# linghuaj/AlphaGo

Measured on AMD Instinct MI355X. Metric: SL-policy positions/sec (whole node) + top-1 move acc, 19x19 12-layer net, higher is better.
Workload: dtype bf16; 1 GPU; model=SL policy net (12-layer, 192 filters, 48 planes), global_batch=2176, per_gpu_batch=2176, seq_len=361, parallelism=dp1, backend=hip, graph=False, wgrad_direct=False, merged_reduce=False

## Files before the change

alphago_amd/_build.py:

```python
from __future__ import annotations

import glob
import hashlib
import os
import subprocess
import sys
import sysconfig
from concurrent.futures import ThreadPoolExecutor

PKG = os.path.dirname(os.path.abspath(__file__))
CSRC = os.path.join(PKG, "csrc")
BUILD = os.path.join(os.path.dirname(PKG), "build", "native")
ROCM = os.environ.get("ROCM_PATH", "/opt/rocm")
ARCH = os.environ.get("PYTORCH_ROCM_ARCH", "gfx950")


def _ext_suffix() -> str:
    return sysconfig.get_config_var("EXT_SUFFIX") or ".so"


def engine_path() -> str:
    return os.path.join(PKG, "_engine" + _ext_suffix())


# ... 75 lines not shown
    return out


def build_selftest(sanitize: str = "", force: bool = False, verbose: bool = False) -> str:
    srcs = sorted(glob.glob(os.path.join(CSRC, "engine", "*.cpp")))
    srcs = [s for s in srcs if not s.endswith(("bindings.cpp", "lzf.cpp", "lockstep.cpp"))]
    hdrs = sorted(glob.glob(os.path.join(CSRC, "engine", "*.h")))
    main = os.path.join(CSRC, "tools", "engine_selftest.cpp")
    tag = sanitize.replace(",", "_") if sanitize else "plain"
    out = os.path.join(BUILD, "engine_selftest_" + tag)
    flags = ["-std=c++17", "-g", "-mpopcnt", "-DAG_NO_PYBIND=1", "-Wall", "-Wno-sign-compare"]
    flags += (["-O1", "-fno-omit-frame-pointer", "-fsanitize=" + sanitize] if sanitize else ["-O2"])
    if sanitize and "undefined" in sanitize:
        flags.append("-fno-sanitize-recover=undefined")
    digest = _digest(srcs + hdrs + [main], " ".join(flags))
    if not force and _up_to_date(out, digest):
        return out
    os.makedirs(BUILD, exist_ok=True)
    _run(["g++", *flags, "-I" + os.path.join(CSRC, "engine"), *srcs, main, "-o", out, "-lpthread"], verbose)
    _write_stamp(out, digest)
    return out


def _torch_paths():
    import torch
    from torch.utils import cpp_extension

    incs = cpp_extension.include_paths(device_type="cuda")
    libdir = os.path.join(os.path.dirname(torch.__file__), "lib")
    abi = "1" if torch._C._GLIBCXX_USE_CXX11_ABI else "0"
    return incs, libdir, abi


def build_hip(force: bool = False, verbose: bool = False, flavor: str = "prod") -> str:
    srcs = _hip_sources(flavor)
    hdrs = sorted(glob.glob(os.path.join(CSRC, "kernels", "*.h")) + [os.path.join(CSRC, "engine", "ladder_bb.h")])
    out = hip_path(flavor)
    incs, libdir, abi = _torch_paths()
    common = [
        "-O3",
        "-std=c++17",
        "-fPIC",
        "-D_GLIBCXX_USE_CXX11_ABI=" + abi,
        "-DUSE_ROCM=1",
        "-D__HIP_PLATFORM_AMD__=1",
        "-DTORCH_EXTENSION_NAME=_hip_kernels",
        "-Wno-unused-result",
        "-Wno-deprecated-declarations",
    ] + {"prod": [], "debug": ["-DAGK_DEBUG=1"],
         "lab": ["-DAGK_KERNEL_LAB=1", "-Dagk=agk_lab", "-Dagk_ops=agk_lab_ops"]}[flavor]
    hip_flags = ["--offload-arch=" + ARCH, "-fgpu-rdc" if False else "-fno-gpu-rdc", "-munsafe-fp-atomics"]
    digest = _digest(srcs + hdrs, " ".join(common + hip_flags))
    if not force and _up_to_date(out, digest):
        return out
    os.makedirs(BUILD, exist_ok=True)
    inc_flags = ["-I" + p for p in incs] + ["-I" + os.path.join(CSRC, "kernels"), "-I" + sysconfig.get_paths()["include"]]
    hipcc = os.path.join(ROCM, "bin", "hipcc")

    def compile_one(src):
        obj = os.path.join(BUILD, "hip_%s_%s.o" % (flavor, os.path.basename(src)))
        cmd = [hipcc, "-x", "hip", *common, *hip_flags, *inc_flags, "-c", src, "-o", obj]
        _run(cmd, verbose)
        return obj

    with ThreadPoolExecutor(max_workers=min(8, max(1, len(srcs)))) as ex:
        objs = list(ex.map(compile_one, srcs))
    tmp = out + ".tmp"
    _run(
        [
            hipcc,
            "-shared",
            "--offload-arch=" + ARCH,
            "-o",
            tmp,
            *objs,
            "-L" + libdir,
            "-Wl,-rpath," + libdir,
            "-lc10",
            "-lc10_hip",
            "-ltorch",
            "-ltorch_cpu",
            "-ltorch_hip",
            "-lamdhip64",
        ],
        verbose,
    )
    os.replace(tmp, out)
    _write_stamp(out, digest)
    return out
# ... 24 lines not shown
```

alphago_amd/csrc/kernels/conv_common.h:

```cpp
#pragma once
#include <hip/hip_runtime.h>

#include <utility>

#include "common.h"
#include "kernels.h"

namespace agk {

#ifdef AGK_DEBUG
static __device__ unsigned g_dbg_err;
#define AGK_DCHECK(cond, code) \
  ((cond) ? true : (atomicOr(&::agk::g_dbg_err, (unsigned)(code)), false))
#else
#define AGK_DCHECK(cond, code) true
#endif
enum : unsigned {
  DBG_FWD_X = 1u << 0,
  DBG_FWD_W = 1u << 1,
  DBG_FWD_Y = 1u << 2,
  DBG_WG_X = 1u << 3,
  DBG_WG_DZ = 1u << 4,
};

// ... 94 lines not shown
  static_assert(OFF >= 0 && OFF < 65536, "ds_read offset: 16-bit unsigned");
  bf16x4 v;
  asm volatile("ds_read_b64_tr_b16 %0, %1 offset:%2" : "=v"(v) : "v"(lds_addr), "n"(OFF));
  return v;
}
template <int OFF = 0>
__device__ __forceinline__ bf16x4 ds_read_tr16_asm(const char* p) {
  return ds_read_tr16_at<OFF>((uint32_t)(uintptr_t)(AG_LDS(p)));
}

__device__ __forceinline__ const char* sgpr_ptr(const char* p) {
  const uint64_t v = (uint64_t)(uintptr_t)p;
  uint32_t lo = __builtin_amdgcn_readfirstlane((uint32_t)v), hi = __builtin_amdgcn_readfirstlane((uint32_t)(v >> 32));
  asm("" : "+s"(lo), "+s"(hi));
  return (const char*)(uintptr_t)(((uint64_t)hi << 32) | lo);
}
__device__ __forceinline__ void glds16_so(const void* sbase, uint32_t voff, void* lds_wave_base) {
  glds16((const char*)sbase + (size_t)voff, lds_wave_base);
}


template <int NB, int MB, int MODE>
struct ConvEpilogue {
  static constexpr int BASE = MODE & 3;
  static constexpr bool RES = (MODE & MODE_RES) != 0;
  static_assert(!RES || BASE == MODE_BIAS_RELU || BASE == MODE_MASKBITS, "skip operand: bias + ReLU or bitmask dgrad");
  static constexpr bool BF8 = BASE == MODE_MASKBITS && !RES;
  static constexpr int RG = !(RES && MB >= 6) ? 1 : (18 / NB < 1 ? 1 : (18 / NB > MB ? MB : 18 / NB));
  int ooff[MB];
  int pix[MB];
  f32x4 bb[NB];
  bf16x4 mk[NB][MB];
  uint32_t mw[MB];
  int mslot, mwords;

  __device__ __forceinline__ void load(const ConvFwdArgs& a, int mrow, int nbase, int wn = 0) {
    const int SS = a.S * a.S;
    mslot = blockIdx.y * 8 + wn * 4 + ((threadIdx.x & 63) >> 4);
    mwords = gridDim.y * 8;
#pragma unroll
    for (int j = 0; j < MB; ++j) {
      int m = mrow + j * 16;
      m = m < a.M ? m : a.M - 1;
      const int b = fdiv(m, a.divSS);
      const int rem = m - b * SS;
      const int ii = fdiv(rem, a.divS);
      const int jj = rem - ii * a.S;
      pix[j] = (b * a.HPo + ii + a.Po) * a.HPo + jj + a.Po;
      ooff[j] = pix[j] * a.Cout + nbase;
    }
    if constexpr (BASE == MODE_BIAS_RELU) {
#pragma unroll
      for (int i = 0; i < NB; ++i) bb[i] = *(const f32x4*)(a.bias + nbase + i * 16);
    } else if constexpr (BASE == MODE_MASK) {
#pragma unroll
      for (int j = 0; j < MB; ++j)
#pragma unroll
        for (int i = 0; i < NB; ++i) mk[i][j] = *(const bf16x4*)(a.mask + ooff[j] + i * 16);
    } else if constexpr (BASE == MODE_MASKBITS) {
#pragma unroll
      for (int j = 0; j < MB; ++j) mw[j] = a.mbits_in[(size_t)pix[j] * mwords + mslot];
    }
  }

  __device__ __forceinline__ void store(const ConvFwdArgs& a, const f32x4 (&acc)[NB][MB], int mrow) const {
    float gmax = 0.f;
    const float gsc = (BF8 && a.y_bf8) ? *a.bf8_scale : 0.f;
    bf16x4 rs[RG][RES ? NB : 1];
#pragma unroll
    for (int j = 0; j < MB; ++j) {
      if constexpr (RES) {
        if (j % RG == 0) {
#pragma unroll
          for (int jg = 0; jg < RG; ++jg)
#pragma unroll
            for (int i = 0; i < NB; ++i)
              if (j + jg < MB) rs[jg][i] = *(const bf16x4*)(a.res + ooff[j + jg < MB ? j + jg : j] + i * 16);
        }
      }
      if (mrow + j * 16 >= a.M) continue;
      uint32_t bits = 0u;
#pragma unroll
      for (int i = 0; i < NB; ++i) {
        f32x4 v = acc[i][j];
        if constexpr (RES) {
#pragma unroll
          for (int r = 0; r < 4; ++r)
            v[r] = (BASE == MODE_BIAS_RELU ? v[r] + bb[i][r] : v[r]) + (float)rs[j % RG][i][r];
        }
        if constexpr (BASE == MODE_BIAS_RELU && RES) {
          v[0] = fmaxf(v[0], 0.f);
          v[1] = fmaxf(v[1], 0.f);
          v[2] = fmaxf(v[2], 0.f);
          v[3] = fmaxf(v[3], 0.f);
        } else if constexpr (BASE == MODE_BIAS_RELU) {
          v[0] = fmaxf(v[0] + bb[i][0], 0.f);
          v[1] = fmaxf(v[1] + bb[i][1], 0.f);
          v[2] = fmaxf(v[2] + bb[i][2], 0.f);
          v[3] = fmaxf(v[3] + bb[i][3], 0.f);
        } else if constexpr (BASE == MODE_MASK) {
          v[0] = (float)mk[i][j][0] > 0.f ? v[0] : 0.f;
          v[1] = (float)mk[i][j][1] > 0.f ? v[1] : 0.f;
          v[2] = (float)mk[i][j][2] > 0.f ? v[2] : 0.f;
          v[3] = (float)mk[i][j][3] > 0.f ? v[3] : 0.f;
        } else if constexpr (BASE == MODE_MASKBITS) {
#pragma unroll
          for (int r = 0; r < 4; ++r) v[r] = ((mw[j] >> (4 * i + r)) & 1u) ? v[r] : 0.f;
        }
        bf16x4 o;
        o[0] = (__bf16)v[0];
        o[1] = (__bf16)v[1];
        o[2] = (__bf16)v[2];
        o[3] = (__bf16)v[3];
        if constexpr (BASE == MODE_BIAS_RELU) {
#pragma unroll
          for (int r = 0; r < 4; ++r) bits |= ((float)o[r] > 0.f ? 1u : 0u) << (4 * i + r);
        }
#ifdef AGK_DEBUG
        const long long yo = (long long)ooff[j] + i * 16;
        if (AGK_DCHECK(yo >= 0 && yo + 4 <= a.y_elems, DBG_FWD_Y)) *(bf16x4*)(a.y + yo) = o;
#else
        *(bf16x4*)(a.y + ooff[j] + i * 16) = o;
#endif
        if constexpr (BF8) {
          if (a.y_bf8) {
            float sv[4];
#pragma unroll
            for (int r = 0; r < 4; ++r) {
              gmax = fmaxf(gmax, fabsf(v[r]));
              sv[r] = fminf(fmaxf(v[r] * gsc, -57344.f), 57344.f);
            }
            int pk = __builtin_amdgcn_cvt_pk_bf8_f32(sv[0], sv[1], 0, false);
            pk = __builtin_amdgcn_cvt_pk_bf8_f32(sv[2], sv[3], pk, true);
            *(int*)(a.y_bf8 + ooff[j] + i * 16) = pk;
          }
        }
      }
      if constexpr (BASE == MODE_BIAS_RELU)
        if (a.mbits_out) a.mbits_out[(size_t)pix[j] * mwords + mslot] = bits;
    }
    if constexpr (BF8) {
      if (a.y_bf8 && a.bf8_amax) {
        gmax = wave_max(gmax);
        if ((threadIdx.x & 63) == 0 && gmax > 0.f) atomicMax(a.bf8_amax + (blockIdx.x & 63), __float_as_uint(gmax));
      }
    }
  }
};

template <int NB, int MB, int MODE>
__device__ __forceinline__ void conv_store_tile(const ConvFwdArgs& a, const f32x4 (&acc)[NB][MB], int mrow,
                                                int nbase, int wn) {
  ConvEpilogue<NB, MB, MODE> ep;
  ep.load(a, mrow, nbase, wn);
  ep.store(a, acc, mrow);
}

template <int NB, int MB, int MODE>
struct ConvEpilogue32 {
  static constexpr int BASE = MODE & 3;
  static constexpr bool RES = (MODE & MODE_RES) != 0;
  static_assert(!RES || BASE == MODE_BIAS_RELU || BASE == MODE_MASKBITS, "skip operand: bias + ReLU or bitmask dgrad");
  int ooff[MB];
  int pix[MB];
  f32x4 bb[NB][4];
  bf16x4 mk[NB][MB][4];
  uint2 mw[MB];
  int mslot, mwords;

  __device__ __forceinline__ void load(const ConvFwdArgs& a, int mrow, int nbase, int wn) {
    const int SS = a.S * a.S;
    const int h = (threadIdx.x & 63) >> 5;
    mslot = blockIdx.y * 8 + wn * 4 + h;
    mwords = gridDim.y * 8;
#pragma unroll
    for (int j = 0; j < MB; ++j) {
      int m = mrow + j * 32;
      m = m < a.M ? m : a.M - 1;
      const int b = fdiv(m, a.divSS);
      const int rem = m - b * SS;
      const int ii = fdiv(rem, a.divS);
      const int jj = rem - ii * a.S;
      pix[j] = (b * a.HPo + ii + a.Po) * a.HPo + jj + a.Po;
      ooff[j] = pix[j] * a.Cout + nbase + 4 * h;
    }
    if constexpr (BASE == MODE_BIAS_RELU) {
#pragma unroll
// ... 76 lines not shown
```

alphago_amd/csrc/kernels/conv_fwd_variants.hip:

```cpp
#include <hip/hip_runtime.h>

#include <algorithm>
#include <numeric>

#include "common.h"
#include "conv_common.h"
#include "kernels.h"

namespace agk {

constexpr int HALO_BM = 256;
constexpr int HALO_ROWS = 320;
constexpr int HALO_PW = HALO_ROWS / 8 / 8;


template <int BN, int MODE>
__global__ __launch_bounds__(512, 1) void conv_fwd_halo_kernel(ConvFwdArgs a) {
  constexpr int NB = BN / 32;
  constexpr int MB = 4;
  constexpr int W_BYTES = BN * 128;
  constexpr int H_BYTES = HALO_ROWS * 128;
  constexpr int NW_PW = BN / 64;
  extern __shared__ __attribute__((aligned(16))) char smem[];
  char* const hbuf = smem;
// ... 387 lines not shown
    asm volatile("s_waitcnt lgkmcnt(0)" ::: "memory");
    if constexpr (STAMP) ts[3] = __builtin_amdgcn_s_memtime();
    __builtin_amdgcn_sched_barrier(0);
    __builtin_amdgcn_s_barrier();
    __builtin_amdgcn_sched_barrier(0);
    if constexpr (STAMP) ts[4] = __builtin_amdgcn_s_memtime();
    __builtin_amdgcn_s_setprio(1);
#pragma unroll
    for (int i = 0; i < NB; ++i)
#pragma unroll
      for (int j = 0; j < MB; ++j) acc[i][j] = mfma16x16x32(wf[i], xf[j], acc[i][j]);
    __builtin_amdgcn_s_setprio(0);
    __builtin_amdgcn_sched_barrier(0);
    if constexpr (STAMP) ts[5] = __builtin_amdgcn_s_memtime();
    __builtin_amdgcn_s_barrier();
    __builtin_amdgcn_sched_barrier(0);
    if constexpr (STAMP) {
      ts[6] = __builtin_amdgcn_s_memtime();
#pragma unroll
      for (int i = 0; i < 6; ++i) st_sum[i] += ts[i + 1] - ts[i];
      st_sum[6] += ts[7] - ts[0];
    }
  }
  if constexpr (STAMP) {
    if (lane == 0) {
      unsigned long long* d = a.dbg + ((size_t)blockIdx.x * 8 + wave) * 8;
#pragma unroll
      for (int i = 0; i < 6; ++i) d[i] = st_sum[i];
      d[6] = __builtin_amdgcn_s_memtime() - st_begin;
      d[7] = nK | (st_sum[6] << 16);
    }
  }
  if (grp == 0) __builtin_amdgcn_s_barrier();
  ep.store(a, acc, ep_mrow);
}


template <int BN, int MODE>
static void launch_fwd_pp(const ConvFwdArgs& a_in, hipStream_t st) {
  constexpr int smem = PP_SLOTS * (PP_BM * 64 + BN * 64);
  if constexpr (BN == 192 && MODE == MODE_BIAS_RELU) {
    if (a_in.dbg) {
      static const hipError_t attr_d = hipFuncSetAttribute((const void*)conv_fwd_pp_kernel<BN, MODE, true>,
                            hipFuncAttributeMaxDynamicSharedMemorySize, smem);
  hip_check(attr_d, "hipFuncSetAttribute(max dynamic LDS)");
      ConvFwdArgs a = a_in;
      dim3 grid((a.M + PP_BM - 1) / PP_BM, a.Cout / BN);
      hipLaunchKernelGGL((conv_fwd_pp_kernel<BN, MODE, true>), grid, dim3(512), smem, st, a);
      return;
    }
  }
  const ConvFwdArgs& a = a_in;
  static const hipError_t attr = hipFuncSetAttribute((const void*)conv_fwd_pp_kernel<BN, MODE>, hipFuncAttributeMaxDynamicSharedMemorySize, smem);
  hip_check(attr, "hipFuncSetAttribute(max dynamic LDS)");
  dim3 grid((a.M + PP_BM - 1) / PP_BM, a.Cout / BN);
  hipLaunchKernelGGL((conv_fwd_pp_kernel<BN, MODE>), grid, dim3(512), smem, st, a);
}

template <int BN, int MODE>
static void launch_fwd_ring(const ConvFwdArgs& a, hipStream_t st) {
  constexpr int smem = RING_SLOTS * (RING_BM * 64 + BN * 64);
  static const hipError_t attr = hipFuncSetAttribute((const void*)conv_fwd_ring_kernel<BN, MODE>, hipFuncAttributeMaxDynamicSharedMemorySize,
                        smem);
  hip_check(attr, "hipFuncSetAttribute(max dynamic LDS)");
  dim3 grid((a.M + RING_BM - 1) / RING_BM, a.Cout / BN);
  hipLaunchKernelGGL((conv_fwd_ring_kernel<BN, MODE>), grid, dim3(512), smem, st, a);
// ... 111 lines not shown
  for (int ks = 0; ks < nK; ++ks) {
    const int tn = (t + 1 == T) ? 0 : t + 1;
    const int cn = (t + 1 == T) ? c + 1 : c;
    if (ks + 1 < nK) stage_w(tn, cn, (ks + 1) & 1);
    if (t == 0 && c + 1 < CC) stage_halo(c + 1, (c + 1) & 1);
    if (ks == (nK > 2 ? nK - 2 : 0)) ep.load(a, ep_mrow, ep_nbase, wn);
    const char* hb = hbuf + (c & 1) * H_BYTES;
    const char* wb = wbuf + (ks & 1) * W_BYTES;
    const int kh = t / a.K, kw = t - (t / a.K) * a.K;
    const int toff = (kh - a.K / 2) * HP + (kw - a.K / 2) + G;
#pragma unroll
    for (int kk = 0; kk < 2; ++kk) {
      const int ch = (kk << 2) + (lane >> 4);
      bf16x8 xf[MB], wf[NB];
#pragma unroll
      for (int j = 0; j < MB; ++j) {
        const int row = qrel[j] + toff - G;
        xf[j] = *(const bf16x8*)(hb + row * 128 + ((ch ^ ((row >> 1) & 7)) << 4));
      }
#pragma unroll
      for (int i = 0; i < NB; ++i) wf[i] = *(const bf16x8*)(wb + wrow0 + i * 16 * 128 + ((ch ^ swzw) << 4));
      __builtin_amdgcn_s_setprio(1);
#pragma unroll
      for (int i = 0; i < NB; ++i)
#pragma unroll
        for (int j = 0; j < MB; ++j) acc[i][j] = mfma16x16x32(wf[i], xf[j], acc[i][j]);
      __builtin_amdgcn_s_setprio(0);
    }
    wait_vmcnt0();
    __syncthreads();
    t = tn;
    c = cn;
  }
  ep.store(a, acc, ep_mrow);
}

template <int BN, int MODE, bool STAMP = false>
__global__ __launch_bounds__(512, 1) void conv_fwd_hpp_kernel(ConvFwdArgs a) {
  uint64_t st_sum[8] = {0, 0, 0, 0, 0, 0, 0, 0}, ts[9];
#define HPP_STAMP(i)                          \
  if constexpr (STAMP) {                      \
    __builtin_amdgcn_sched_barrier(0);        \
    ts[i] = __builtin_amdgcn_s_memtime();     \
    __builtin_amdgcn_sched_barrier(0);        \
  }
  constexpr int NB = BN / 32;
  constexpr int MB = 4;
  constexpr int H_BYTES = HC_ROWS * 128;
  constexpr int W_BYTES = BN * 128;
  constexpr int WP = BN / 32;
  constexpr int H_PIECES = HC_DATA / 8;
  constexpr int HP1 = H_PIECES / 4;
  constexpr int HP_STEP = 2;
  constexpr int T = 9;
  static_assert(HP1 == 5 * HP_STEP && H_PIECES % 8 == 0, "halo pieces must be issued within steps 0..4");
  extern __shared__ __attribute__((aligned(16))) char smem[];
  char* const hbuf = smem;
  char* const wbuf = smem + 2 * H_BYTES;

  const int lane = threadIdx.x & 63;
  const int wave = wave_id();
  const int grp = wave >> 2;
  const int wq = wave & 3;
  const int wm = grp * 2 + ((wave >> 1) & 1);
  const int wn = wave & 1;
  const int nwg = gridDim.x;
// ... 134 lines not shown
    __builtin_amdgcn_sched_group_barrier(0x008, NB * MB - 2 * (MB + NB), 0);
    asm volatile("s_waitcnt lgkmcnt(0)" ::: "memory");
    __builtin_amdgcn_sched_barrier(0);
#pragma unroll
    for (int i = 0; i < NB; ++i)
#pragma unroll
      for (int j = 0; j < MB; ++j) acc[i][j] = mfma16x16x32(wf[1][i], xf[1][j], acc[i][j]);
    __builtin_amdgcn_s_setprio(0);
    HPP_STAMP(5);
    __builtin_amdgcn_sched_barrier(0);
    if (grp == 0) wait_vmcnt0();
    HPP_STAMP(6);
    __builtin_amdgcn_sched_barrier(0);
    __builtin_amdgcn_s_barrier();
    __builtin_amdgcn_sched_barrier(0);
    HPP_STAMP(7);
    if constexpr (STAMP) {
#pragma unroll
      for (int i = 0; i < 7; ++i) st_sum[i] += ts[i + 1] - ts[i];
    }
    t = tn; c = cn; kh = khn; kw = kwn;
    wslot = wslot == 2 ? 0 : wslot + 1;
  }
  if constexpr (STAMP) {
    if (lane == 0) {
      unsigned long long* d = a.dbg + ((size_t)blockIdx.x * 8 + wave) * 8;
#pragma unroll
      for (int i = 0; i < 7; ++i) d[i] = st_sum[i];
      d[7] = __builtin_amdgcn_s_memtime() - st_begin;
    }
  }
#undef HPP_STAMP
  if (grp == 0) __builtin_amdgcn_s_barrier();
  ep.store(a, acc, ep_mrow);
}

constexpr int H32_DATA3 = 320;
constexpr int H32_DATA5 = 344;

template <int BN, int MODE, int K, bool STAMP = false>
__global__ __launch_bounds__(512, 1) void conv_fwd_h32_kernel(ConvFwdArgs a) {
  uint64_t st_sum[8] = {0, 0, 0, 0, 0, 0, 0, 0}, ts[9];
#define H32_STAMP(i)                          \
  if constexpr (STAMP) {                      \
    __builtin_amdgcn_sched_barrier(0);        \
    ts[i] = __builtin_amdgcn_s_memtime();     \
    __builtin_amdgcn_sched_barrier(0);        \
  }
  constexpr int NB = BN / 64;
  constexpr int MB = 2;
  constexpr int T = K * K;
  constexpr int HDATA = K == 3 ? H32_DATA3 : H32_DATA5;
  constexpr int HROWS = HDATA + 16;
  constexpr int NHBUF = K == 3 ? 2 : 1;
  constexpr int H_BYTES = HROWS * 128;
  constexpr int W_BYTES = BN * 128;
  constexpr int WP = BN / 64;
  constexpr int H_PIECES = HDATA / 8;
  constexpr int HP1 = H_PIECES / 4;
  constexpr int HP_STEP = 2;
  static_assert(K == 5 || HP1 == 5 * HP_STEP, "K=3 halo pieces are issued in steps 0..4");
  extern __shared__ __attribute__((aligned(16))) char smem[];
  char* const hbuf = smem;
  char* const wbuf = smem + NHBUF * H_BYTES;

  const int lane = threadIdx.x & 63;
// ... 337 lines not shown
```

alphago_amd/csrc/kernels/conv_kernels.h:

```cpp
#pragma once
#include <hip/hip_runtime.h>

#include <stdexcept>

#include "common.h"
#include "conv_common.h"
#include "kernels.h"

namespace agk {

template <int BN, int MODE, int BM, int MBW, bool EPF = true, bool PIPE = true, bool M32 = false, bool ILV = false,
          bool STR = false, bool CO = false, int NS = 2, bool SK = false>
__global__ __launch_bounds__(BM / MBW * 8, 1) void conv_fwd_kernel(ConvFwdArgs a) {
  constexpr int NW = BM / (16 * MBW) * 2;
  constexpr int NB = BN / 32;
  constexpr int MB = MBW;
  constexpr int A_BYTES = BM * 128;
  constexpr int B_BYTES = BN * 128;
  constexpr int STAGE = A_BYTES + B_BYTES;
  constexpr int A_ROWS_PW = BM / NW;
  constexpr int A_INSTR = A_ROWS_PW / 8;
  constexpr bool BDIST = (BN / NW) % 8 != 0;
  constexpr int B_ROWS_PW = BN / NW;
  constexpr int B_INSTR = BDIST ? (BN / 8 + NW - 1) / NW : B_ROWS_PW / 8;
// ... 137 lines not shown
  auto mfmas = [&](const bf16x8 (&xf)[MB], const bf16x8 (&wf)[NB]) {
#pragma unroll
    for (int i = 0; i < NB; ++i)
#pragma unroll
      for (int j = 0; j < MB; ++j) acc[i][j] = mfma16x16x32(wf[i], xf[j], acc[i][j]);
  };

  bf16x8 xa[MB], wa[NB], xb[MB], wb[NB];
  const int ep_mrow = m0 + wm * 16 * MB + (lane & 15);
  const int ep_nbase = n0 + wn * (BN / 2) + ((lane >> 4) << 2);
  ConvEpilogue<NB, MB, MODE> ep;
  const int ep_at = EPF ? (nK > 2 ? nK - 2 : 0) : nK - 1;
  if constexpr (NS > 2) {
    static_assert(PIPE && !M32 && !ILV && !BDIST, "ring: the pipelined 16x16 loop");
    constexpr int PW = A_INSTR + B_INSTR;
    static_assert(PW * (NS - 2) <= 63, "vmcnt range");
#pragma unroll
    for (int s = 0; s < NS - 1; ++s)
      if (s < nK) stage(s);
    for (int ks = 0; ks < nK; ++ks) {
      const int later = (nK - 1 - ks) < (NS - 2) ? (nK - 1 - ks) : (NS - 2);
      ring_wait<PW, NS - 2>(later);
      __syncthreads();
      if (ks + NS - 1 < nK) stage((ks + NS - 1) % NS);
      const char* base = smem + (ks % NS) * STAGE;
      read_frags(base, 0, xa, wa);
      read_frags(base, 1, xb, wb);
      if (ks == ep_at) ep.load(a, ep_mrow, ep_nbase, wn);
      __builtin_amdgcn_s_setprio(1);
      mfmas(xa, wa);
      mfmas(xb, wb);
      __builtin_amdgcn_s_setprio(0);
    }
    ep.store(a, acc, ep_mrow);
    return;
  }
  if constexpr (SK) {
    static_assert(PIPE && !M32 && !ILV && !CO, "split-K: the pipelined 2-buffer loop, tap-outer order");
    const int z = blockIdx.z, nz = gridDim.z;
    const int kb = (int)((long)nK * z / nz), ke = (int)((long)nK * (z + 1) / nz);
    for (int i = 0; i < kb; ++i) st_advance();
    if (kb < ke) {
      stage(0);
      wait_vmcnt0();
      __syncthreads();
      read_frags(smem, 0, xa, wa);
      for (int ks = kb; ks < ke; ++ks) {
        const int cur = (ks - kb) & 1;
        const char* base = smem + cur * STAGE;
        if (ks + 1 < ke) stage(cur ^ 1);
        read_frags(base, 1, xb, wb);
        __builtin_amdgcn_sched_barrier(0);
        __builtin_amdgcn_s_setprio(1);
        mfmas(xa, wa);
        mfmas(xb, wb);
        __builtin_amdgcn_s_setprio(0);
        __builtin_amdgcn_sched_barrier(0);
        wait_vmcnt0();
        __syncthreads();
        if (ks + 1 < ke) read_frags(smem + (cur ^ 1) * STAGE, 0, xa, wa);
      }
    }
    float* ws = a.sk_ws + (size_t)z * a.M * a.Cout;
#pragma unroll
    for (int j = 0; j < MB; ++j) {
      const int m = ep_mrow + j * 16;
// ... 77 lines not shown
      int xo0, xo1;
      size_t wo0, wo1;
      st_offsets(xo0, xo1, wo0, wo1);
      xo0 = more ? xo0 : lxo0;
      xo1 = more ? xo1 : lxo1;
      wo0 = more ? wo0 : lwo0;
      wo1 = more ? wo1 : lwo1;
      lxo0 = xo0;
      lxo1 = xo1;
      lwo0 = wo0;
      lwo1 = wo1;
      asm volatile("s_waitcnt lgkmcnt(0)" ::: "memory");
      __builtin_amdgcn_sched_barrier(0);
      __builtin_amdgcn_s_setprio(1);
#pragma unroll
      for (int d = 0; d < NDMA; ++d) {
        mfma_range(d * MPD, (d + 1) * MPD);
        __builtin_amdgcn_sched_barrier(0);
        st_piece(d, nb, xo0, xo1, wo0, wo1);
        __builtin_amdgcn_sched_barrier(0);
      }
      mfma_range(NDMA * MPD, NMF);
      __builtin_amdgcn_s_setprio(0);
      __builtin_amdgcn_sched_barrier(0);
      st_advance();
      read_frags(base, 1, xa, wa);
      __builtin_amdgcn_s_setprio(1);
      mfmas(xa, wa);
      __builtin_amdgcn_s_setprio(0);
      wait_vmcnt0();
      __syncthreads();
    }
    ep.load(a, ep_mrow, ep_nbase, wn);
    ep.store(a, acc, ep_mrow);
    return;
  }
  if constexpr (!PIPE) {
    for (int ks = 0; ks < nK; ++ks) {
      const int cur = ks & 1;
      const char* base = smem + cur * STAGE;
      if (ks + 1 < nK) stage(cur ^ 1);
#pragma unroll
      for (int kk = 0; kk < 2; ++kk) {
        read_frags(base, kk, xa, wa);
        __builtin_amdgcn_s_setprio(1);
        mfmas(xa, wa);
        __builtin_amdgcn_s_setprio(0);
      }
      wait_vmcnt0();
      __syncthreads();
    }
    ep.load(a, ep_mrow, ep_nbase, wn);
    ep.store(a, acc, ep_mrow);
    return;
  }
  read_frags(smem, 0, xa, wa);
  for (int ks = 0; ks < nK; ++ks) {
    const int cur = ks & 1;
    const char* base = smem + cur * STAGE;
    if (ks + 1 < nK) stage(cur ^ 1);
    if (ks == ep_at) ep.load(a, ep_mrow, ep_nbase, wn);
    read_frags(base, 1, xb, wb);
    __builtin_amdgcn_sched_barrier(0);
    __builtin_amdgcn_s_setprio(1);
    mfmas(xa, wa);
    mfmas(xb, wb);
    __builtin_amdgcn_s_setprio(0);
    __builtin_amdgcn_sched_barrier(0);
    wait_vmcnt0();
    __syncthreads();
    if (ks + 1 < nK) read_frags(base + (cur ^ 1) * STAGE - cur * STAGE, 0, xa, wa);
  }

  ep.store(a, acc, ep_mrow);
}

template <int BN, int MODE, int BM, int MBW, bool EPF = true, bool PIPE = true, bool M32 = false, bool ILV = false,
          bool STR = false, bool CO = false, int NS = 2>
static void launch_fwd_bm(const ConvFwdArgs& a, hipStream_t st) {
  constexpr int smem = NS * (BM * 128 + BN * 128);
  static_assert(smem <= 160 * 1024, "LDS");
  static const hipError_t attr = hipFuncSetAttribute(
      (const void*)conv_fwd_kernel<BN, MODE, BM, MBW, EPF, PIPE, M32, ILV, STR, CO, NS>,
      hipFuncAttributeMaxDynamicSharedMemorySize, smem);
  hip_check(attr, "hipFuncSetAttribute(max dynamic LDS)");
  dim3 grid((a.M + BM - 1) / BM, a.Cout / BN);
  hipLaunchKernelGGL((conv_fwd_kernel<BN, MODE, BM, MBW, EPF, PIPE, M32, ILV, STR, CO, NS>), grid,
                     dim3(BM / MBW * 8), smem, st, a);
}

constexpr int H384_BM = 384;
constexpr int H384_SMAX = 19;
constexpr int H384_DATA = (H384_BM + 2 * (H384_SMAX + 1) + 7) / 8 * 8;
constexpr int H384_ROWS = H384_DATA + 8;
constexpr int H384_PIECES = H384_DATA / 8;

template <int V>
struct IntC {
  static constexpr int value = V;
};

template <int BN, int MODE>
__global__ __launch_bounds__(512, 1) void conv_fwd_halo384_kernel(ConvFwdArgs a) {
  constexpr int BM = H384_BM, MB = 6, NW = 8;
  constexpr int NB = BN / 32;
  constexpr int NMF = NB * MB;
  constexpr int H_BYTES = H384_ROWS * 128;
  constexpr int W_BYTES = BN * 128;
  constexpr int WP = BN / 8 / NW;
  constexpr int HPW = (H384_PIECES + NW - 1) / NW;
  static_assert(BN % 64 == 0 && BM == NW / 2 * 16 * MB, "tile geometry");
  static_assert(2 * H_BYTES + 2 * W_BYTES <= 160 * 1024, "LDS: two halo buffers and two weight slots, S <= 19");
  static_assert(HPW <= 7, "the next chunk's halo is issued in the first seven taps");
  extern __shared__ __attribute__((aligned(16))) char smem[];
  char* const hbuf = smem;
  char* const wbuf = smem + 2 * H_BYTES;

  const int lane = threadIdx.x & 63;
  const int wave = wave_id();
  const int wm = wave >> 1, wn = wave & 1;
  const int m0 = blockIdx.x * BM;
  const int n0 = blockIdx.y * BN;
  const int S = a.S;
  const int SS = S * S;
  const int CC = a.Cin >> 6;
  const int G = S + 1;
  const int Pc = a.offi + 1;

  int hoff[HPW];
#pragma unroll
  for (int i = 0; i < HPW; ++i) {
    const int k = i * NW + wave < H384_PIECES ? i * NW + wave : H384_PIECES - 1;
    const int r = k * 8 + (lane >> 3);
    int m = m0 - G + r;
    m = m < 0 ? 0 : (m >= a.M ? a.M - 1 : m);
    const int b = fdiv(m, a.divSS);
    const int rem = m - b * SS;
    const int ii = fdiv(rem, a.divS);
    const int q = (b * a.HPi + ii + Pc) * a.HPi + (rem - ii * S) + Pc;
    hoff[i] = q * a.Cin + (((lane & 7) ^ ((r >> 1) & 7)) << 3);
  }
  auto halo_piece = [&](int i, int c, int buf) {
    const int k = i * NW + wave < H384_PIECES ? i * NW + wave : H384_PIECES - 1;
    const int xo = hoff[i] + c * 64;
#ifdef AGK_DEBUG
    const bool ok = AGK_DCHECK(xo >= 0 && (long long)xo + 8 <= a.x_elems, DBG_FWD_X);
    glds16(a.x + (ok ? xo : 0), hbuf + buf * H_BYTES + k * 1024);
#else
    glds16(a.x + xo, hbuf + buf * H_BYTES + k * 1024);
#endif
// ... 95 lines not shown
    }
    mfma_range(NDMA * MPD, NMF);
    __builtin_amdgcn_s_setprio(0);
    __builtin_amdgcn_sched_barrier(0);
#pragma unroll
    for (int j = 0; j < MB; ++j) xa[j] = *(const bf16x8*)(hb + (xo[j] ^ 64));
#pragma unroll
    for (int i = 0; i < NB; ++i) wa[i] = *(const bf16x8*)(wbuf + ws * W_BYTES + (wfrag0 ^ 64) + i * 16 * 128);
    __builtin_amdgcn_s_setprio(1);
    mfma_range(0, NMF);
    __builtin_amdgcn_s_setprio(0);
    wait_vmcnt0();
    __syncthreads();
    ws ^= 1;
  };
  auto chunk = [&](auto nc, int c) {
    step(IntC<0>{}, nc, c);
    step(IntC<1>{}, nc, c);
    step(IntC<2>{}, nc, c);
    step(IntC<3>{}, nc, c);
    step(IntC<4>{}, nc, c);
    step(IntC<5>{}, nc, c);
    step(IntC<6>{}, nc, c);
    step(IntC<7>{}, nc, c);
    step(IntC<8>{}, nc, c);
  };
  for (int c = 0; c + 1 < CC; ++c) chunk(IntC<1>{}, c);
  chunk(IntC<0>{}, CC - 1);

  int ep_mrow = m0 + wm * 16 * MB + pix16;
  asm volatile("" : "+v"(ep_mrow));
  const int ep_nbase = n0 + wn * (BN / 2) + ((lane >> 4) << 2);
  ConvEpilogue<NB, MB, MODE> ep;
  ep.load(a, ep_mrow, ep_nbase, wn);
  ep.store(a, acc, ep_mrow);
}

template <int BN, int MODE>
static bool halo384_covers(const ConvFwdArgs& a) {
  return BN == 192 && ((MODE & 3) == MODE_BIAS_RELU || (MODE & 3) == MODE_MASKBITS) && a.K == 3 && a.Cin % 64 == 0 &&
         a.Cin >= 64 && a.S <= H384_SMAX && a.offi >= 0 && 9ll * a.Cout * a.Cin < (1ll << 31);
}

template <int BN, int MODE>
static void launch_fwd_halo384(const ConvFwdArgs& a, hipStream_t st) {
  if constexpr (BN == 192 && ((MODE & 3) == MODE_BIAS_RELU || (MODE & 3) == MODE_MASKBITS)) {
    constexpr int smem = 2 * H384_ROWS * 128 + 2 * BN * 128;
    static const hipError_t attr = hipFuncSetAttribute((const void*)conv_fwd_halo384_kernel<BN, MODE>,
                                                       hipFuncAttributeMaxDynamicSharedMemorySize, smem);
    hip_check(attr, "hipFuncSetAttribute(max dynamic LDS)");
    dim3 grid((a.M + H384_BM - 1) / H384_BM, a.Cout / BN);
    hipLaunchKernelGGL((conv_fwd_halo384_kernel<BN, MODE>), grid, dim3(512), smem, st, a);
  } else {
    throw std::invalid_argument("conv_fwd: tile 388 is the 192-wide forward / bitmask dgrad");
  }
}

template <int MODE, int NB>
__global__ __launch_bounds__(256) void conv_splitk_finish_kernel(ConvFwdArgs a) {
  constexpr int BN = 32 * NB;
  constexpr int BASE = MODE & 3;
  constexpr bool RES = (MODE & MODE_RES) != 0;
  const int WPP = (a.Cout / BN) * 8;
  const long gid = (long)blockIdx.x * 256 + threadIdx.x;
  if (gid >= (long)a.M * WPP) return;
  const int m = (int)(gid / WPP), w = (int)(gid - (long)m * WPP);
  const int base = (w >> 3) * BN + ((w >> 2) & 1) * (BN / 2) + 4 * (w & 3);
  f32x4 v[NB];
#pragma unroll
  for (int i = 0; i < NB; ++i) v[i] = f32x4{0.f, 0.f, 0.f, 0.f};
  for (int z = 0; z < a.sk_nsplit; ++z) {
    const float* src = a.sk_ws + ((size_t)z * a.M + m) * a.Cout + base;
#pragma unroll
    for (int i = 0; i < NB; ++i) v[i] += *(const f32x4*)(src + 16 * i);
  }
  const int SS = a.S * a.S;
  const int b = fdiv(m, a.divSS);
  const int rem = m - b * SS;
  const int ii = fdiv(rem, a.divS);
  const int jj = rem - ii * a.S;
  const size_t pix = (size_t)(b * a.HPo + ii + a.Po) * a.HPo + jj + a.Po;
  uint32_t mw = 0u, bits = 0u;
  if constexpr (BASE == MODE_MASKBITS) mw = a.mbits_in[pix * WPP + w];
#pragma unroll
// ... 148 lines not shown
  const int swz = (lane & 15) >> 1;
  const int xrow0 = (wm * 16 * MB + (lane & 15)) * 128;
  const int wrow0 = A_BYTES + (wn * (BN / 2) + (lane & 15)) * 128;
  bf16x8 xf[MB], wf[NB];
  ConvEpilogue<NB, MB, MODE_BIAS_RELU> ep;
  const int ep_mrow = m0 + wm * 16 * MB + (lane & 15);
  const int ep_nbase = n0 + wn * (BN / 2) + ((lane >> 4) << 2);

  stage(0);
  wait_vmcnt0();
  __syncthreads();
  for (int ks = 0; ks < nK; ++ks) {
    const int cur = ks & 1;
    const char* base = smem + cur * STAGE;
    if (ks + 1 < nK) stage(cur ^ 1);
#pragma unroll
    for (int kk = 0; kk < 2; ++kk) {
      const int choff = (((kk << 2) + (lane >> 4)) ^ swz) << 4;
#pragma unroll
      for (int j = 0; j < MB; ++j) xf[j] = *(const bf16x8*)(base + xrow0 + j * 16 * 128 + choff);
#pragma unroll
      for (int i = 0; i < NB; ++i) wf[i] = *(const bf16x8*)(base + wrow0 + i * 16 * 128 + choff);
      __builtin_amdgcn_s_setprio(1);
#pragma unroll
      for (int i = 0; i < NB; ++i)
#pragma unroll
        for (int j = 0; j < MB; ++j) acc[i][j] = mfma16x16x32(wf[i], xf[j], acc[i][j]);
      __builtin_amdgcn_s_setprio(0);
    }
    wait_vmcnt0();
    __syncthreads();
  }
  ep.load(a, ep_mrow, ep_nbase, wn);
  ep.store(a, acc, ep_mrow);
}


template <int WN, int WC, int NWC, int TAPS, int NWN = 2>
__device__ __forceinline__ void wgrad_store(const ConvWgradArgs& a,
                                            const f32x4 (&acc)[TAPS][WN / (16 * NWN)][WC / (16 * NWC)],
                                            const float (&dbs)[WN / (16 * NWN)], unsigned bmask, int split, int t,
                                            int n0, int c0, int wn, int wc, int lane, int zero_split) {
  constexpr int NBn = WN / (16 * NWN), NBc = WC / (16 * NWC);
  const int nb0 = n0 + wn * (WN / NWN) + ((lane >> 4) << 2);
  const int cbase = c0 + wc * (WC / NWC) + (lane & 15);
  if (a.grad_w) {
    const float sc = a.scale, be = a.beta;
#pragma unroll
    for (int tp = 0; tp < TAPS; ++tp)
#pragma unroll
      for (int i = 0; i < NBn; ++i)
#pragma unroll
        for (int j = 0; j < NBc; ++j) {
          const int c = cbase + j * 16;
#pragma unroll
          for (int r = 0; r < 4; ++r) {
            const int n = nb0 + i * 16 + r;
            if (n < a.cout_real && c < a.cin_real) {
              float* g = a.grad_w + ((size_t)n * a.cin_real + c) * a.T + t + tp;
              *g = (be != 0.f ? be * *g : 0.f) + sc * acc[tp][i][j][r];
            }
          }
        }
    if (bmask && a.grad_b) {
#pragma unroll
      for (int i = 0; i < NBn; ++i) {
// ... 628 lines not shown
```

alphago_amd/csrc/kernels/conv_lab.hip:

```cpp
#include <hip/hip_runtime.h>

#include "conv_kernels.h"

namespace agk {

template <int BN, int MODE>
__global__ __launch_bounds__(512, 1) void conv_fwd_ga_kernel(ConvFwdArgs a) {
  constexpr int MB = 3;
  constexpr int NB = BN / 16;
  constexpr int NH = NB / 2;
  constexpr int BM = 8 * 16 * MB;
  constexpr int W_BYTES = BN * 128;
  constexpr int WPIECES = BN / 8;
  constexpr int WPW = (WPIECES + 7) / 8;
  static_assert(NB % 2 == 0, "two channel halves");
  extern __shared__ __attribute__((aligned(16))) char smem[];

  const int lane = threadIdx.x & 63;
  const int wave = wave_id();
  const int nwg = gridDim.x;
  const int xcd = blockIdx.x & 7, q8 = nwg >> 3, r8 = nwg & 7;
  const int tile = (xcd < r8 ? xcd * (q8 + 1) : r8 * (q8 + 1) + (xcd - r8) * q8) + (blockIdx.x >> 3);
  const int m0 = tile * BM;
  const int n0 = blockIdx.y * BN;
// ... 82 lines not shown
      const int ch = ((kk << 2) + (lane >> 4)) ^ swz;
#pragma unroll
      for (int h = 0; h < 2; ++h) {
        bf16x8 wf[NH];
#pragma unroll
        for (int i = 0; i < NH; ++i) wf[i] = *(const bf16x8*)(wb + wr0 + (h * NH + i) * 16 * 128 + (ch << 4));
        __builtin_amdgcn_s_setprio(1);
#pragma unroll
        for (int i = 0; i < NH; ++i)
#pragma unroll
          for (int j = 0; j < MB; ++j) acc[h * NH + i][j] = mfma16x16x32(wf[i], x[kk][j], acc[h * NH + i][j]);
        __builtin_amdgcn_s_setprio(0);
      }
      __builtin_amdgcn_sched_barrier(0);
      load_x(x[kk], kk);
      __builtin_amdgcn_sched_barrier(0);
    }
    advance();
    store_w((ks + 1) & 1);
    __syncthreads();
  }
  wait_vmcnt0();

  const int mrow = m0 + wave * 16 * MB + (lane & 15);
#pragma unroll
  for (int h = 0; h < 2; ++h) {
    f32x4 ah[NH][MB];
#pragma unroll
    for (int i = 0; i < NH; ++i)
#pragma unroll
      for (int j = 0; j < MB; ++j) ah[i][j] = acc[h * NH + i][j];
    ConvEpilogue<NH, MB, MODE> ep;
    ep.load(a, mrow, n0 + h * (BN / 2) + ((lane >> 4) << 2), h);
    ep.store(a, ah, mrow);
  }
}

template <int BN, int MODE>
static void launch_fwd_ga(const ConvFwdArgs& a, hipStream_t st) {
  constexpr int smem = 2 * BN * 128;
  static const hipError_t attr = hipFuncSetAttribute((const void*)conv_fwd_ga_kernel<BN, MODE>, hipFuncAttributeMaxDynamicSharedMemorySize, smem);
  hip_check(attr, "hipFuncSetAttribute(max dynamic LDS)");
  constexpr int BM = 8 * 16 * 3;
  dim3 grid((a.M + BM - 1) / BM, a.Cout / BN);
  hipLaunchKernelGGL((conv_fwd_ga_kernel<BN, MODE>), grid, dim3(512), smem, st, a);
}


template <int WN, int WC, int WRING_SLOTS>
__global__ __launch_bounds__(512, 1) void conv_wgrad_ring_kernel(ConvWgradArgs a) {
  constexpr int AHEAD = WRING_SLOTS - 1;
  constexpr int NBn = WN / 32;
  constexpr int NBc = WC / 64;
  constexpr int DZ_BYTES = WN * 64;
  constexpr int X_BYTES = WC * 64;
  constexpr int SLOT = DZ_BYTES + X_BYTES;
  constexpr int NINSTR = (WN + WC) / 16;
  constexpr int IPW = (NINSTR + 7) / 8;
  extern __shared__ __attribute__((aligned(16))) char smem[];

  const int lane = threadIdx.x & 63;
  const int wave = wave_id();
  const int wn = wave >> 2, wc = wave & 3;
  const int split = blockIdx.x;
  const int t = blockIdx.y;
  const int ncb = a.Cin / WC;
// ... 245 lines not shown
```

Measured before the change: 137,300 positions/s.

## Widen conv epilogue stores via permlane16 swap and hoist epilogue branching

The forward conv epilogue now pairs adjacent channel blocks and uses permlane16_swap so each lane writes 16-byte (and 8-byte bf8) stores instead of 8-byte (4-byte) ones, halving store instruction count. Runtime branches on y_bf8/mbits_out are hoisted out of the per-element loop into templated store_rows variants, and a settle() step pins epilogue loads in registers before the store phase (with bf8 scale made scalar via readfirstlane). A lab-only timestamp probe variant of the halo384 kernel is added, plus a build-flag refactor. Risks include extra register pressure and changed store address patterns.

```diff
diff --git a/alphago_amd/_build.py b/alphago_amd/_build.py
--- a/alphago_amd/_build.py
+++ b/alphago_amd/_build.py
@@ -131,10 +131,7 @@
     return incs, libdir, abi
 
 
-def build_hip(force: bool = False, verbose: bool = False, flavor: str = "prod") -> str:
-    srcs = _hip_sources(flavor)
-    hdrs = sorted(glob.glob(os.path.join(CSRC, "kernels", "*.h")) + [os.path.join(CSRC, "engine", "ladder_bb.h")])
-    out = hip_path(flavor)
+def hip_compile_flags(flavor: str = "prod"):
     incs, libdir, abi = _torch_paths()
     common = [
         "-O3",
@@ -149,11 +146,19 @@
     ] + {"prod": [], "debug": ["-DAGK_DEBUG=1"],
          "lab": ["-DAGK_KERNEL_LAB=1", "-Dagk=agk_lab", "-Dagk_ops=agk_lab_ops"]}[flavor]
     hip_flags = ["--offload-arch=" + ARCH, "-fgpu-rdc" if False else "-fno-gpu-rdc", "-munsafe-fp-atomics"]
+    inc_flags = ["-I" + p for p in incs] + ["-I" + os.path.join(CSRC, "kernels"), "-I" + sysconfig.get_paths()["include"]]
+    return common, hip_flags, inc_flags, libdir
+
+
+def build_hip(force: bool = False, verbose: bool = False, flavor: str = "prod") -> str:
+    srcs = _hip_sources(flavor)
+    hdrs = sorted(glob.glob(os.path.join(CSRC, "kernels", "*.h")) + [os.path.join(CSRC, "engine", "ladder_bb.h")])
+    out = hip_path(flavor)
+    common, hip_flags, inc_flags, libdir = hip_compile_flags(flavor)
     digest = _digest(srcs + hdrs, " ".join(common + hip_flags))
     if not force and _up_to_date(out, digest):
         return out
     os.makedirs(BUILD, exist_ok=True)
-    inc_flags = ["-I" + p for p in incs] + ["-I" + os.path.join(CSRC, "kernels"), "-I" + sysconfig.get_paths()["include"]]
     hipcc = os.path.join(ROCM, "bin", "hipcc")
 
     def compile_one(src):
diff --git a/alphago_amd/csrc/kernels/conv_common.h b/alphago_amd/csrc/kernels/conv_common.h
--- a/alphago_amd/csrc/kernels/conv_common.h
+++ b/alphago_amd/csrc/kernels/conv_common.h
@@ -150,6 +150,7 @@
   f32x4 bb[NB];
   bf16x4 mk[NB][MB];
   uint32_t mw[MB];
+  float gsc;
   int mslot, mwords;
 
   __device__ __forceinline__ void load(const ConvFwdArgs& a, int mrow, int nbase, int wn = 0) {
@@ -178,13 +179,105 @@
     } else if constexpr (BASE == MODE_MASKBITS) {
 #pragma unroll
       for (int j = 0; j < MB; ++j) mw[j] = a.mbits_in[(size_t)pix[j] * mwords + mslot];
-    }
-  }
+      if constexpr (BF8) gsc = a.y_bf8 ? *a.bf8_scale : 0.f;
+    }
+  }
+
+  __device__ __forceinline__ void settle() {
+    if constexpr (RES) return;
+    if constexpr (BASE == MODE_BIAS_RELU) {
+#pragma unroll
+      for (int i = 0; i < NB; ++i) asm volatile("" : "+v"(bb[i]));
+    } else if constexpr (BASE == MODE_MASK) {
+#pragma unroll
+      for (int i = 0; i < NB; ++i)
+#pragma unroll
+        for (int j = 0; j < MB; ++j) asm volatile("" : "+v"(mk[i][j]));
+    } else if constexpr (BASE == MODE_MASKBITS) {
+#pragma unroll
+      for (int j = 0; j < MB; ++j) asm volatile("" : "+v"(mw[j]));
+      if constexpr (BF8) {
+        asm volatile("" : "+v"(gsc));
+        gsc = __uint_as_float(__builtin_amdgcn_readfirstlane(__float_as_uint(gsc)));
+      }
+    }
+  }
+
+  static constexpr int NBP = RES ? 0 : NB;
+  typedef uint32_t u32x4_a8 __attribute__((ext_vector_type(4), aligned(8)));
+  typedef uint32_t u32x2_a4 __attribute__((ext_vector_type(2), aligned(4)));
 
   __device__ __forceinline__ void store(const ConvFwdArgs& a, const f32x4 (&acc)[NB][MB], int mrow) const {
     float gmax = 0.f;
-    const float gsc = (BF8 && a.y_bf8) ? *a.bf8_scale : 0.f;
+    if constexpr (BF8) {
+      if (a.y_bf8) store_rows<0, true>(a, acc, mrow, gmax);
+      else store_rows<0, false>(a, acc, mrow, gmax);
+      if (a.y_bf8 && a.bf8_amax) {
+        gmax = wave_max(gmax);
+        if ((threadIdx.x & 63) == 0 && gmax > 0.f) atomicMax(a.bf8_amax + (blockIdx.x & 63), __float_as_uint(gmax));
+      }
+    } else if constexpr (BASE == MODE_BIAS_RELU && RES) {
+      store_rows<2, false>(a, acc, mrow, gmax);
+    } else if constexpr (BASE == MODE_BIAS_RELU) {
+      if (a.mbits_out) store_rows<1, false>(a, acc, mrow, gmax);
+      else store_rows<0, false>(a, acc, mrow, gmax);
+    } else {
+      store_rows<0, false>(a, acc, mrow, gmax);
+    }
+  }
+
+  template <int BITS, bool E5M2>
+  __device__ __forceinline__ void store_rows(const ConvFwdArgs& a, const f32x4 (&acc)[NB][MB], int mrow,
+                                             float& gmax) const {
+    const int po = (threadIdx.x & 16) ? 12 : 0;
     bf16x4 rs[RG][RES ? NB : 1];
+    auto block = [&](int i, int j, uint2& ow, uint32_t& pk, uint32_t& bits) {
+      f32x4 v = acc[i][j];
+      if constexpr (RES) {
+#pragma unroll
+        for (int r = 0; r < 4; ++r)
+          v[r] = (BASE == MODE_BIAS_RELU ? v[r] + bb[i][r] : v[r]) + (float)rs[j % RG][i][r];
+      }
+      if constexpr (BASE == MODE_BIAS_RELU && RES) {
+        v[0] = fmaxf(v[0], 0.f);
+        v[1] = fmaxf(v[1], 0.f);
+        v[2] = fmaxf(v[2], 0.f);
+        v[3] = fmaxf(v[3], 0.f);
+      } else if constexpr (BASE == MODE_BIAS_RELU) {
+        v[0] = fmaxf(v[0] + bb[i][0], 0.f);
+        v[1] = fmaxf(v[1] + bb[i][1], 0.f);
+        v[2] = fmaxf(v[2] + bb[i][2], 0.f);
+        v[3] = fmaxf(v[3] + bb[i][3], 0.f);
+      } else if constexpr (BASE == MODE_MASK) {
+        v[0] = (float)mk[i][j][0] > 0.f ? v[0] : 0.f;
+        v[1] = (float)mk[i][j][1] > 0.f ? v[1] : 0.f;
+        v[2] = (float)mk[i][j][2] > 0.f ? v[2] : 0.f;
+        v[3] = (float)mk[i][j][3] > 0.f ? v[3] : 0.f;
+      } else if constexpr (BASE == MODE_MASKBITS) {
+#pragma unroll
+        for (int r = 0; r < 4; ++r) v[r] = ((mw[j] >> (4 * i + r)) & 1u) ? v[r] : 0.f;
+      }
+      bf16x4 o;
+      o[0] = (__bf16)v[0];
+      o[1] = (__bf16)v[1];
+      o[2] = (__bf16)v[2];
+      o[3] = (__bf16)v[3];
+      if constexpr (BASE == MODE_BIAS_RELU) {
+#pragma unroll
+        for (int r = 0; r < 4; ++r) bits |= ((float)o[r] > 0.f ? 1u : 0u) << (4 * i + r);
+      }
+      ow = __builtin_bit_cast(uint2, o);
+      if constexpr (E5M2) {
+        float sv[4];
+#pragma unroll
+        for (int r = 0; r < 4; ++r) {
+          gmax = fmaxf(gmax, fabsf(v[r]));
+          sv[r] = fminf(fmaxf(v[r] * gsc, -57344.f), 57344.f);
+        }
+        int p = __builtin_amdgcn_cvt_pk_bf8_f32(sv[0], sv[1], 0, false);
+        pk = (uint32_t)__builtin_amdgcn_cvt_pk_bf8_f32(sv[2], sv[3], p, true);
+      }
+    };
 #pragma unroll
     for (int j = 0; j < MB; ++j) {
       if constexpr (RES) {
@@ -199,69 +292,47 @@
       if (mrow + j * 16 >= a.M) continue;
       uint32_t bits = 0u;
 #pragma unroll
-      for (int i = 0; i < NB; ++i) {
-        f32x4 v = acc[i][j];
-        if constexpr (RES) {
-#pragma unroll
-          for (int r = 0; r < 4; ++r)
-            v[r] = (BASE == MODE_BIAS_RELU ? v[r] + bb[i][r] : v[r]) + (float)rs[j % RG][i][r];
+      for (int i = 0; i + 1 < NBP; i += 2) {
+        uint2 o0, o1;
+        uint32_t p0 = 0u, p1 = 0u;
+        block(i, j, o0, p0, bits);
+        block(i + 1, j, o1, p1, bits);
+        const auto sx = __builtin_amdgcn_permlane16_swap(o0.x, o1.x, false, false);
+        const auto sy = __builtin_amdgcn_permlane16_swap(o0.y, o1.y, false, false);
+        u32x4_a8 q;
+        q[0] = sx[0];
+        q[1] = sy[0];
+        q[2] = sx[1];
+        q[3] = sy[1];
+#ifdef AGK_DEBUG
+        const long long yo = (long long)ooff[j] + i * 16 + po;
+        if (AGK_DCHECK(yo >= 0 && yo + 8 <= a.y_elems, DBG_FWD_Y)) *(u32x4_a8*)(a.y + yo) = q;
+#else
+        *(u32x4_a8*)(a.y + ooff[j] + i * 16 + po) = q;
+#endif
+        if constexpr (E5M2) {
+          const auto sp = __builtin_amdgcn_permlane16_swap(p0, p1, false, false);
+          u32x2_a4 q8;
+          q8[0] = sp[0];
+          q8[1] = sp[1];
+          *(u32x2_a4*)(a.y_bf8 + ooff[j] + i * 16 + po) = q8;
         }
-        if constexpr (BASE == MODE_BIAS_RELU && RES) {
-          v[0] = fmaxf(v[0], 0.f);
-          v[1] = fmaxf(v[1], 0.f);
-          v[2] = fmaxf(v[2], 0.f);
-          v[3] = fmaxf(v[3], 0.f);
-        } else if constexpr (BASE == MODE_BIAS_RELU) {
-          v[0] = fmaxf(v[0] + bb[i][0], 0.f);
-          v[1] = fmaxf(v[1] + bb[i][1], 0.f);
-          v[2] = fmaxf(v[2] + bb[i][2], 0.f);
-          v[3] = fmaxf(v[3] + bb[i][3], 0.f);
-        } else if constexpr (BASE == MODE_MASK) {
-          v[0] = (float)mk[i][j][0] > 0.f ? v[0] : 0.f;
-          v[1] = (float)mk[i][j][1] > 0.f ? v[1] : 0.f;
-          v[2] = (float)mk[i][j][2] > 0.f ? v[2] : 0.f;
-          v[3] = (float)mk[i][j][3] > 0.f ? v[3] : 0.f;
-        } else if constexpr (BASE == MODE_MASKBITS) {
-#pragma unroll
-          for (int r = 0; r < 4; ++r) v[r] = ((mw[j] >> (4 * i + r)) & 1u) ? v[r] : 0.f;
-        }
-        bf16x4 o;
-        o[0] = (__bf16)v[0];
-        o[1] = (__bf16)v[1];
-        o[2] = (__bf16)v[2];
-        o[3] = (__bf16)v[3];
-        if constexpr (BASE == MODE_BIAS_RELU) {
-#pragma unroll
-          for (int r = 0; r < 4; ++r) bits |= ((float)o[r] > 0.f ? 1u : 0u) << (4 * i + r);
-        }
+      }
+#pragma unroll
+      for (int i = NBP / 2 * 2; i < NB; ++i) {
+        uint2 o0;
+        uint32_t p0 = 0u;
+        block(i, j, o0, p0, bits);
 #ifdef AGK_DEBUG
         const long long yo = (long long)ooff[j] + i * 16;
-        if (AGK_DCHECK(yo >= 0 && yo + 4 <= a.y_elems, DBG_FWD_Y)) *(bf16x4*)(a.y + yo) = o;
+        if (AGK_DCHECK(yo >= 0 && yo + 4 <= a.y_elems, DBG_FWD_Y)) *(uint2*)(a.y + yo) = o0;
 #else
-        *(bf16x4*)(a.y + ooff[j] + i * 16) = o;
+        *(uint2*)(a.y + ooff[j] + i * 16) = o0;
 #endif
-        if constexpr (BF8) {
-          if (a.y_bf8) {
-            float sv[4];
-#pragma unroll
-            for (int r = 0; r < 4; ++r) {
-              gmax = fmaxf(gmax, fabsf(v[r]));
-              sv[r] = fminf(fmaxf(v[r] * gsc, -57344.f), 57344.f);
-            }
-            int pk = __builtin_amdgcn_cvt_pk_bf8_f32(sv[0], sv[1], 0, false);
-            pk = __builtin_amdgcn_cvt_pk_bf8_f32(sv[2], sv[3], pk, true);
-            *(int*)(a.y_bf8 + ooff[j] + i * 16) = pk;
-          }
-        }
-      }
-      if constexpr (BASE == MODE_BIAS_RELU)
-        if (a.mbits_out) a.mbits_out[(size_t)pix[j] * mwords + mslot] = bits;
-    }
-    if constexpr (BF8) {
-      if (a.y_bf8 && a.bf8_amax) {
-        gmax = wave_max(gmax);
-        if ((threadIdx.x & 63) == 0 && gmax > 0.f) atomicMax(a.bf8_amax + (blockIdx.x & 63), __float_as_uint(gmax));
-      }
+        if constexpr (E5M2) *(uint32_t*)(a.y_bf8 + ooff[j] + i * 16) = p0;
+      }
+      if constexpr (BITS != 0)
+        if (BITS == 1 || a.mbits_out) a.mbits_out[(size_t)pix[j] * mwords + mslot] = bits;
     }
   }
 };
@@ -271,6 +342,7 @@
                                                 int nbase, int wn) {
   ConvEpilogue<NB, MB, MODE> ep;
   ep.load(a, mrow, nbase, wn);
+  ep.settle();
   ep.store(a, acc, mrow);
 }
 
diff --git a/alphago_amd/csrc/kernels/conv_fwd_variants.hip b/alphago_amd/csrc/kernels/conv_fwd_variants.hip
--- a/alphago_amd/csrc/kernels/conv_fwd_variants.hip
+++ b/alphago_amd/csrc/kernels/conv_fwd_variants.hip
@@ -443,6 +443,7 @@
     }
   }
   if (grp == 0) __builtin_amdgcn_s_barrier();
+  ep.settle();
   ep.store(a, acc, ep_mrow);
 }
 
@@ -620,6 +621,7 @@
     t = tn;
     c = cn;
   }
+  ep.settle();
   ep.store(a, acc, ep_mrow);
 }
 
@@ -820,6 +822,7 @@
   }
 #undef HPP_STAMP
   if (grp == 0) __builtin_amdgcn_s_barrier();
+  ep.settle();
   ep.store(a, acc, ep_mrow);
 }
 
diff --git a/alphago_amd/csrc/kernels/conv_kernels.h b/alphago_amd/csrc/kernels/conv_kernels.h
--- a/alphago_amd/csrc/kernels/conv_kernels.h
+++ b/alphago_amd/csrc/kernels/conv_kernels.h
@@ -193,6 +193,7 @@
       mfmas(xb, wb);
       __builtin_amdgcn_s_setprio(0);
     }
+    ep.settle();
     ep.store(a, acc, ep_mrow);
     return;
   }
@@ -336,6 +337,7 @@
       __syncthreads();
     }
     ep.load(a, ep_mrow, ep_nbase, wn);
+    ep.settle();
     ep.store(a, acc, ep_mrow);
     return;
   }
@@ -355,6 +357,7 @@
       __syncthreads();
     }
     ep.load(a, ep_mrow, ep_nbase, wn);
+    ep.settle();
     ep.store(a, acc, ep_mrow);
     return;
   }
@@ -376,6 +379,7 @@
     if (ks + 1 < nK) read_frags(base + (cur ^ 1) * STAGE - cur * STAGE, 0, xa, wa);
   }
 
+  ep.settle();
   ep.store(a, acc, ep_mrow);
 }
 
@@ -404,7 +408,7 @@
   static constexpr int value = V;
 };
 
-template <int BN, int MODE>
+template <int BN, int MODE, bool STAMP = false>
 __global__ __launch_bounds__(512, 1) void conv_fwd_halo384_kernel(ConvFwdArgs a) {
   constexpr int BM = H384_BM, MB = 6, NW = 8;
   constexpr int NB = BN / 32;
@@ -420,6 +424,8 @@
   char* const hbuf = smem;
   char* const wbuf = smem + 2 * H_BYTES;
 
+  unsigned long long t_begin = 0;
+  if constexpr (STAMP) t_begin = __builtin_amdgcn_s_memtime();
   const int lane = threadIdx.x & 63;
   const int wave = wave_id();
   const int wm = wave >> 1, wn = wave & 1;
@@ -581,7 +587,31 @@
   asm volatile("" : "+v"(ep_mrow));
   const int ep_nbase = n0 + wn * (BN / 2) + ((lane >> 4) << 2);
   ConvEpilogue<NB, MB, MODE> ep;
+  if constexpr (STAMP) {
+    __builtin_amdgcn_sched_barrier(0);
+    const unsigned long long t0 = __builtin_amdgcn_s_memtime();
+    __builtin_amdgcn_sched_barrier(0);
+    ep.load(a, ep_mrow, ep_nbase, wn);
+    ep.settle();
+    __builtin_amdgcn_sched_barrier(0);
+    const unsigned long long t1 = __builtin_amdgcn_s_memtime();
+    __builtin_amdgcn_sched_barrier(0);
+    ep.store(a, acc, ep_mrow);
+    __builtin_amdgcn_sched_barrier(0);
+    const unsigned long long t2 = __builtin_amdgcn_s_memtime();
+    wait_vmcnt0();
+    const unsigned long long t3 = __builtin_amdgcn_s_memtime();
+    if (lane == 0) {
+      unsigned long long* d = a.dbg + ((size_t)(blockIdx.y * gridDim.x + blockIdx.x) * NW + wave) * 4;
+      d[0] = t1 - t0;
+      d[1] = t2 - t0;
+      d[2] = t3 - t0;
+      d[3] = t3 - t_begin;
+    }
+    return;
+  }
   ep.load(a, ep_mrow, ep_nbase, wn);
+  ep.settle();
   ep.store(a, acc, ep_mrow);
 }
 
@@ -599,6 +629,15 @@
                                                        hipFuncAttributeMaxDynamicSharedMemorySize, smem);
     hip_check(attr, "hipFuncSetAttribute(max dynamic LDS)");
     dim3 grid((a.M + H384_BM - 1) / H384_BM, a.Cout / BN);
+#ifdef AGK_KERNEL_LAB
+    if (a.dbg) {
+      static const hipError_t attr_d = hipFuncSetAttribute((const void*)conv_fwd_halo384_kernel<BN, MODE, true>,
+                                                           hipFuncAttributeMaxDynamicSharedMemorySize, smem);
+      hip_check(attr_d, "hipFuncSetAttribute(max dynamic LDS)");
+      hipLaunchKernelGGL((conv_fwd_halo384_kernel<BN, MODE, true>), grid, dim3(512), smem, st, a);
+      return;
+    }
+#endif
     hipLaunchKernelGGL((conv_fwd_halo384_kernel<BN, MODE>), grid, dim3(512), smem, st, a);
   } else {
     throw std::invalid_argument("conv_fwd: tile 388 is the 192-wide forward / bitmask dgrad");
@@ -813,6 +852,7 @@
     __syncthreads();
   }
   ep.load(a, ep_mrow, ep_nbase, wn);
+  ep.settle();
   ep.store(a, acc, ep_mrow);
 }
 
diff --git a/alphago_amd/csrc/kernels/conv_lab.hip b/alphago_amd/csrc/kernels/conv_lab.hip
--- a/alphago_amd/csrc/kernels/conv_lab.hip
+++ b/alphago_amd/csrc/kernels/conv_lab.hip
@@ -138,6 +138,7 @@
       for (int j = 0; j < MB; ++j) ah[i][j] = acc[h * NH + i][j];
     ConvEpilogue<NH, MB, MODE> ep;
     ep.load(a, mrow, n0 + h * (BN / 2) + ((lane >> 4) << 2), h);
+    ep.settle();
     ep.store(a, ah, mrow);
   }
 }
```

Measured after the change: 141,800 positions/s (median of 6 runs). 3.3% higher.
